# sjtuytc/betapose

Measured on AMD Instinct MI355X. Metric: frames/sec (640x480, 50-kp KPD), higher is better.
Workload: dtype f32 as an exact 3-way bf16 operand split (6 bf16 MFMA products), f32 accumulate and activations

## Files before the change

betapose_amd/_lib.py:

```python
from __future__ import annotations

import ctypes as C
import os
import threading

_HERE = os.path.dirname(os.path.abspath(__file__))
LIB_PATH = os.environ.get("BP_LIB") or os.path.join(_HERE, "libbetapose_hip.so")
_lock = threading.Lock()
_lib = None

c_float_p = C.POINTER(C.c_float)
c_double_p = C.POINTER(C.c_double)
c_int_p = C.POINTER(C.c_int)
vp = C.c_void_p

PROTOTYPES = {
    "bp_last_error": (C.c_char_p, []),
    "bp_version": (C.c_int, []),
    "bp_device_count": (C.c_int, []),
    "bp_device_name": (C.c_int, [C.c_int, C.c_char_p, C.c_int]),
    "bp_yolo_create": (C.c_int, [C.c_char_p, C.c_char_p, C.c_int, C.c_int, C.c_int, C.POINTER(vp)]),
    "bp_yolo_create_from_memory": (C.c_int, [C.c_char_p, vp, C.c_size_t, C.c_int, C.c_int, C.c_int, C.POINTER(vp)]),
    "bp_yolo_clone": (C.c_int, [vp, C.POINTER(vp)]),
    "bp_kpd_clone": (C.c_int, [vp, C.POINTER(vp)]),
# ... 10 lines not shown
    "bp_kpd_destroy": (None, [vp]),
    "bp_kpd_forward": (C.c_int, [vp, vp, C.c_int, vp, vp]),
    "bp_kpd_forward_argmax": (C.c_int, [vp, vp, C.c_int, vp, vp, vp]),
    "bp_kpd_tap_count": (C.c_int, [vp]),
    "bp_kpd_tap_info": (C.c_int, [vp, C.c_int, C.c_char_p, C.c_int, c_int_p, c_int_p, c_int_p]),
    "bp_kpd_tap_copy": (C.c_int, [vp, C.c_int, C.c_int, vp, vp]),
    "bp_yolo_set_policy": (C.c_int, [vp, C.c_int, C.c_int, C.c_int, C.c_int]),
    "bp_kpd_set_policy": (C.c_int, [vp, C.c_int, C.c_int, C.c_int, C.c_int]),
    "bp_yolo_set_precision": (C.c_int, [vp, C.c_int]),
    "bp_kpd_set_precision": (C.c_int, [vp, C.c_int]),
    "bp_calibrate_ticks": (C.c_int, [C.c_longlong, c_float_p, vp]),
    "bp_yolo_set_prefetch": (C.c_int, [vp, C.c_int]),
    "bp_kpd_set_prefetch": (C.c_int, [vp, C.c_int]),
    "bp_yolo_set_fusion": (C.c_int, [vp, C.c_int]),
    "bp_kpd_set_fusion": (C.c_int, [vp, C.c_int]),
    "bp_yolo_fused_launches": (C.c_int, [vp, C.c_int, C.POINTER(C.c_int)]),
    "bp_kpd_fused_launches": (C.c_int, [vp, C.c_int, C.POINTER(C.c_int)]),
    "bp_yolo_xcd_errors": (C.c_int, [vp, C.POINTER(C.c_int), vp]),
    "bp_kpd_xcd_errors": (C.c_int, [vp, C.POINTER(C.c_int), vp]),
    "bp_yolo_set_stamps": (C.c_int, [vp, vp, C.c_int]),
    "bp_kpd_set_stamps": (C.c_int, [vp, vp, C.c_int]),
    "bp_yolo_op_name": (C.c_int, [vp, C.c_int, C.c_char_p, C.c_int]),
    "bp_kpd_op_name": (C.c_int, [vp, C.c_int, C.c_char_p, C.c_int]),
    "bp_yolo_op_stats": (C.c_int, [vp, c_double_p, c_double_p, C.c_int]),
    "bp_kpd_op_stats": (C.c_int, [vp, c_double_p, c_double_p, C.c_int]),
    "bp_yolo_device_bytes": (C.c_size_t, [vp]),
    "bp_kpd_device_bytes": (C.c_size_t, [vp]),
    "bp_crop": (C.c_int, [vp, C.c_int, C.c_int, C.c_int, vp, C.c_int, vp, vp, vp, vp, C.c_int, C.c_int, vp]),
    "bp_resize_bicubic": (C.c_int, [vp, C.c_int, C.c_int, C.c_int, C.c_int, C.c_int, C.c_int, vp, vp, vp]),
    "bp_conv2d": (C.c_int, [vp, C.c_int, C.c_int, C.c_int, C.c_int, vp, vp, C.c_int, C.c_int, C.c_int, C.c_int,
# ... 118 lines not shown
```

betapose_amd/csrc/aux_kernels.hip:

```cpp
#include "bp_common.h"

namespace bp {

__device__ __forceinline__ void store_plane(unsigned short* planes, long long idx, long long plane_elems, int np, float v) {
    if (np == 1) {
        const _Float16 h = (_Float16)v;
        planes[idx] = __builtin_bit_cast(unsigned short, h);
    } else if (np == 3) {
        const __bf16 h1 = (__bf16)v;
        const float r1 = v - (float)h1;
        const __bf16 h2 = (__bf16)r1;
        const __bf16 h3 = (__bf16)(r1 - (float)h2);
        planes[idx] = __builtin_bit_cast(unsigned short, h1);
        planes[idx + plane_elems] = __builtin_bit_cast(unsigned short, h2);
        planes[idx + 2 * plane_elems] = __builtin_bit_cast(unsigned short, h3);
    }
}

static inline int grid_for(long long n, int block = 256, int cap = 4096) {
    BP_CHECK(n < (1ll << 31), "tensor too large for 32-bit indexing");
    long long g = (n + block - 1) / block;
    return (int)(g < 1 ? 1 : (g > cap ? cap : g));
}

// ... 243 lines not shown
        const float stride = (float)(reso / g);
        const float* t = H.t + ((long long)n * g * g + cell) * (3 * attrs) + a * attrs;
        float* o = pred + e * attrs;
        o[0] = (sigmoidf_(t[0]) + (float)gx) * stride;
        o[1] = (sigmoidf_(t[1]) + (float)gy) * stride;
        o[2] = (expf(t[2]) * (H.aw[a] / stride)) * stride;
        o[3] = (expf(t[3]) * (H.ah[a] / stride)) * stride;
        for (int k = 4; k < attrs; ++k) o[k] = sigmoidf_(t[k]);
    }
}
void launch_yolo_decode(const YoloHead* heads, int nheads, int N, int reso, int attrs, int rows, float* pred,
                        hipStream_t s) {
    BP_CHECK(nheads <= 4, "at most 4 yolo heads");
    YoloHeads hs;
    hs.n = nheads;
    for (int i = 0; i < nheads; ++i) hs.h[i] = heads[i];
    hipLaunchKernelGGL(yolo_decode_kernel, dim3(grid_for((long long)N * rows)), dim3(256), 0, s, hs, N, reso, attrs, rows, pred);
}

__global__ __launch_bounds__(1024) void yolo_select_kernel(const float* __restrict__ pred, int rows, int attrs,
                                                            float conf, int num_classes, float* __restrict__ sel, int sel_ld) {
    __shared__ float sv[16];
    __shared__ int si[16];
    const int n = blockIdx.x;
    const float* P = pred + (long long)n * rows * attrs;
    const int ncls = min(num_classes, attrs - 5);
    float best = -1.f;
    int bi = 0x7fffffff;
    for (int r = threadIdx.x; r < rows; r += blockDim.x) {
        const float* q = P + (long long)r * attrs;
        const float obj = q[4];
// ... 32 lines not shown
            o[7] = 0.f;
        }
    }
}
void launch_yolo_select(const float* pred, int N, int rows, int attrs, float conf, int num_classes, float* sel,
                        hipStream_t s, int sel_ld) {
    hipLaunchKernelGGL(yolo_select_kernel, dim3(N), dim3(1024), 0, s, pred, rows, attrs, conf, num_classes, sel, sel_ld);
}

__global__ __launch_bounds__(1024) void yolo_decode_select_kernel(YoloHeads hs, int reso, int attrs, int rows, float conf, int num_classes,
                                                                   float* __restrict__ sel, int sel_ld) {
    __shared__ float sv[16];
    __shared__ int si[16];
    const int n = blockIdx.x;
    const int ncls = min(num_classes, attrs - 5);
    auto locate = [&](int row, int* a) -> const float* {
        int hi = 0;
        for (int k = 1; k < hs.n; ++k)
            if (row >= hs.h[k].row_off) hi = k;
        const YoloHead& H = hs.h[hi];
        const int g = H.g, r = row - H.row_off;
        *a = r / (g * g);
        const int cell = r - *a * g * g;
        return H.t + ((long long)n * g * g + cell) * (3 * attrs) + *a * attrs;
    };
    float best = -1.f;
    int bi = 0x7fffffff;
    for (int r = threadIdx.x; r < rows; r += blockDim.x) {
        int a;
        const float* t = locate(r, &a);
        const float obj = sigmoidf_(t[4]);
        if (!(obj > conf)) continue;
        int cls = 0;
        float cm = sigmoidf_(t[5]);
        for (int k = 1; k < ncls; ++k) {
            const float v = sigmoidf_(t[5 + k]);
            if (v > cm) { cm = v; cls = k; }
        }
        if (cls != 0) continue;
        if (obj > best || (obj == best && r < bi)) { best = obj; bi = r; }
    }
    for (int off = 32; off > 0; off >>= 1) {
        const float ov = __shfl_down(best, off, 64);
        const int oi = __shfl_down(bi, off, 64);
        if (ov > best || (ov == best && oi < bi)) { best = ov; bi = oi; }
    }
    const int w = threadIdx.x >> 6;
    if ((threadIdx.x & 63) == 0) { sv[w] = best; si[w] = bi; }
    __syncthreads();
    if (threadIdx.x == 0) {
        for (int k = 1; k < (int)(blockDim.x >> 6); ++k)
            if (sv[k] > best || (sv[k] == best && si[k] < bi)) { best = sv[k]; bi = si[k]; }
        float* o = sel + (long long)n * sel_ld;
        if (best < 0.f) {
            o[0] = __int_as_float(-1);
            for (int k = 1; k < 8; ++k) o[k] = 0.f;
        } else {
            int a, hi = 0;
            const float* t = locate(bi, &a);
            for (int k = 1; k < hs.n; ++k)
                if (bi >= hs.h[k].row_off) hi = k;
            const YoloHead& H = hs.h[hi];
            const int g = H.g, r = bi - H.row_off, cell = r - a * g * g;
            const int gy = cell / g, gx = cell - gy * g;
            const float stride = (float)(reso / g);
            const float q0 = (sigmoidf_(t[0]) + (float)gx) * stride;
            const float q1 = (sigmoidf_(t[1]) + (float)gy) * stride;
            const float q2 = (expf(t[2]) * (H.aw[a] / stride)) * stride;
            const float q3 = (expf(t[3]) * (H.ah[a] / stride)) * stride;
            o[0] = __int_as_float(bi);
            o[1] = q0 - q2 / 2;
            o[2] = q1 - q3 / 2;
            o[3] = q0 + q2 / 2;
            o[4] = q1 + q3 / 2;
            o[5] = sigmoidf_(t[4]);
            o[6] = sigmoidf_(t[5]);
            o[7] = 0.f;
        }
    }
}
void launch_yolo_decode_select(const YoloHead* heads, int nheads, int N, int reso, int attrs, int rows, float conf, int num_classes,
                               float* sel, hipStream_t s, int sel_ld) {
    BP_CHECK(nheads <= 4, "at most 4 yolo heads");
    YoloHeads hs;
    hs.n = nheads;
    for (int i = 0; i < nheads; ++i) hs.h[i] = heads[i];
    hipLaunchKernelGGL(yolo_decode_select_kernel, dim3(N), dim3(1024), 0, s, hs, reso, attrs, rows, conf, num_classes, sel, sel_ld);
}

__global__ __launch_bounds__(256) void heatmap_argmax_kernel(const float* __restrict__ hm, int H, int W,
                                                              float* __restrict__ out, int C, int out_ld) {
    __shared__ float sv[4];
    __shared__ int si[4];
    const int HW = H * W;
    const float* P = hm + (long long)blockIdx.x * HW;
    float best = -INFINITY;
    int bi = 0x7fffffff;
    for (int i = threadIdx.x; i < HW; i += 256) {
        const float v = P[i];
        if (v > best) { best = v; bi = i; }
    }
// ... 270 lines not shown
```

betapose_amd/csrc/bp_common.h:

```cpp
#pragma once
#include <hip/hip_runtime.h>
#include <cstdint>
#include <cstdio>
#include <mutex>
#include <set>
#include <stdexcept>
#include <string>
#include <utility>

namespace bp {

struct Error : std::runtime_error {
    using std::runtime_error::runtime_error;
};

#define BP_HIP(expr)                                                                      \
    do {                                                                                  \
        hipError_t _e = (expr);                                                           \
        if (_e != hipSuccess)                                                             \
            throw ::bp::Error(std::string(#expr) + ": " + hipGetErrorString(_e) + " @" +  \
                              __FILE__ + ":" + std::to_string(__LINE__));                 \
    } while (0)

#define BP_CHECK(cond, msg)                                                               \
// ... 79 lines not shown
    const unsigned short* wbd;
    const unsigned short* wpl;
    float* pool_out;
    int hy_full, hy_splits, hy_cps;
    int xcd_home;
    int* xcc_of;
    int* err_word;
    int* tickets_local;
    int mtiles, n_tiles;
    int work_blocks;
    const void* pf_ptr;
    int pf_first;
    int pf_ntn, pf_splits, pf_cps, pf_nchunks;
    int pf_tile_stride, pf_chunk_bytes;
    int pf_cap;
};

enum Precision : int { PREC_F32 = 0, PREC_F16 = 1, PREC_BF16X3 = 2, PREC_F16_RES = 3 };

enum ConvTile : int { TILE_64x64 = 0, TILE_128x64 = 1, TILE_W64_1x1 = 2, TILE_W64_1x2 = 3, TILE_W64_2x1 = 5, TILE_W64_2x2 = 6,
                      TILE_KG1 = 7, TILE_KG2 = 8, TILE_KG4 = 9,
                      TILE_RD4 = 10, TILE_RD8 = 11,
                      TILE_64x64_BD = 12,
                      TILE_PL64 = 13,
                      TILE_PL128 = 14,
                      TILE_PL128x64 = 15,
                      TILE_PL256x128 = 16,
                      TILE_STEM3 = 20,
                      TILE_PL64BD = 19,
                      TILE_PL64K2 = 18,
                      TILE_PL128S = 17,
// ... 79 lines not shown
                long long pixels, int C, hipStream_t s);
void launch_upsample2(const float* in, int in_ld, float* out, int out_ld, int N, int H, int W, int C, hipStream_t s);
void launch_copy_channels(const float* in, int in_ld, float* out, int out_ld, long long pixels, int C, hipStream_t s);
void launch_pixel_shuffle2(const float* in, float* out, int N, int H, int W, int C, hipStream_t s,
                           unsigned short* planes = nullptr, long long plane_elems = 0, int np = 0);
int avgpool_parts(int HW);
void launch_avgpool(const float* in, int in_ld, float* out, int N, int HW, int C, hipStream_t s);
void launch_fc(const float* in, const float* w, const float* bias, float* out, int N, int Cin, int Cout,
               int act, int in_parts, float in_scale, hipStream_t s);

struct YoloHead {
    const float* t;
    int g;
    float aw[3], ah[3];
    int row_off;
};
void launch_yolo_decode(const YoloHead* heads, int nheads, int N, int reso, int attrs, int rows,
                        float* pred, hipStream_t s);
void launch_yolo_select(const float* pred, int N, int rows, int attrs, float conf, int num_classes,
                        float* sel, hipStream_t s, int sel_ld = 8);
void launch_yolo_decode_select(const YoloHead* heads, int nheads, int N, int reso, int attrs, int rows, float conf, int num_classes,
                               float* sel, hipStream_t s, int sel_ld = 8);
void launch_heatmap_argmax(const float* hm, int N, int C, int H, int W, float* out, hipStream_t s, int out_ld = 0);

void launch_f32_to_f16(const float* in, unsigned short* out, long long n, hipStream_t s);
void launch_f32_to_bf16x3(const float* in, unsigned short* out_planes, long long n, hipStream_t s);
void launch_f32_to_f16_staged(const float* in, unsigned short* out, int CoutPad, int Kpad, hipStream_t s);
void launch_f32_to_bf16x3_staged(const float* in, unsigned short* out, int CoutPad, int Kpad, hipStream_t s, int Cin_pl = 0);
void launch_probe_placement(int* d_out, int blocks, hipStream_t s);
void launch_spin_ticks(long long ticks, hipStream_t s);
// ... 17 lines not shown
```

betapose_amd/csrc/c_api.cpp:

```cpp
#include "../../include/betapose_hip.h"

#include <algorithm>
#include <cmath>
#include <cstdlib>
#include <cstring>
#include <fstream>
#include <memory>
#include <sstream>
#include <vector>

#include "engine.h"
#include "frame_io.h"

namespace bp {
int solve_pnp(const double* P, const double* U, int n, const double* K, double* R, double* t);
int solve_pnp_refined(const double* P, const double* U, int n, const double* K, double* R, double* t);
int solve_pnp_ransac(const double* P, const double* U, int n, const double* K, double reproj_err, int max_trials,
                     double confidence, double* R, double* t, unsigned char* inlier_mask);
void pnp_ransac_samples(int n, int max_trials, int* idx);
void pnp_ransac_trials_needed(int n, double confidence, int* need);
int pose_nms(const float* bboxes, const float* bbox_scores, const float* preds, const float* scores, int n, int K,
             int* out_pick, float* out_pose, float* out_score, float* out_prop);
int pose_error_blocks(int n);
void launch_pose_errors(const double* model, int n, const double* gt, const double* est, int P, const double* K,
// ... 229 lines not shown
    if (default_precision() != bp::PREC_F32) y->net->set_precision(default_precision());
    *out = y.release();
    return 0;
    BP_CATCH
}

int bp_yolo_clone(const bp_yolo* y, bp_yolo** out) {
    BP_TRY
    BP_CHECK(y && out, "null argument");
    BP_HIP(hipSetDevice(y->device));
    std::unique_ptr<bp_yolo> c(new bp_yolo);
    c->device = y->device;
    c->net.reset(y->net->clone());
    if (y->net->precision() != bp::PREC_F32) c->net->set_precision(y->net->precision_id());
    c->net->set_fusion(y->net->fusion());
    *out = c.release();
    return 0;
    BP_CATCH
}
void bp_yolo_destroy(bp_yolo* y) { delete y; }
int bp_yolo_rows(const bp_yolo* y) { return y ? y->net->rows() : -1; }
int bp_yolo_attrs(const bp_yolo* y) { return y ? y->net->attrs() : -1; }

int bp_yolo_forward(bp_yolo* y, const float* d_img, int batch, float* d_pred, void* stream) {
    BP_TRY
    BP_CHECK(y && d_img && d_pred, "null argument");
    y->net->forward(d_img, false, batch, d_pred, 0.f, 0, nullptr, (hipStream_t)stream);
    return 0;
    BP_CATCH
}
// ... 154 lines not shown
    bp::launch_spin_ticks(1000, s);
    BP_HIP(hipEventRecord(e0, s));
    bp::launch_spin_ticks(ticks, s);
    BP_HIP(hipEventRecord(e1, s));
    BP_HIP(hipEventSynchronize(e1));
    BP_HIP(hipEventElapsedTime(ms, e0, e1));
    (void)hipEventDestroy(e0);
    (void)hipEventDestroy(e1);
    return 0;
    BP_CATCH
}
int bp_yolo_set_prefetch(bp_yolo* y, int on) { y->net->set_prefetch(on != 0); return 0; }
int bp_kpd_set_prefetch(bp_kpd* k, int on) { k->net->set_prefetch(on != 0); return 0; }
int bp_yolo_set_fusion(bp_yolo* y, int on) { y->net->set_fusion(on != 0); return 0; }
int bp_kpd_set_fusion(bp_kpd* k, int on) { k->net->set_fusion(on != 0); return 0; }
int bp_yolo_fused_launches(bp_yolo* y, int batch, int* launches) {
    BP_TRY
    BP_CHECK(y && launches && batch >= 1 && batch <= y->net->max_batch(), "arguments");
    BP_HIP(hipSetDevice(y->device));
    *launches = y->net->fused_launches(batch);
    return 0;
    BP_CATCH
}
int bp_kpd_fused_launches(bp_kpd* k, int batch, int* launches) {
    BP_TRY
    BP_CHECK(k && launches && batch >= 1 && batch <= k->net->max_batch(), "arguments");
    BP_HIP(hipSetDevice(k->device));
    *launches = k->net->fused_launches(batch);
    return 0;
    BP_CATCH
// ... 770 lines not shown
```

betapose_amd/csrc/conv_halo.hip:

```cpp
#include "conv_dev.h"

namespace bp {

static constexpr int HALO_ROW_B = 208;

template <int NW, int NPASS>
__global__ __launch_bounds__(64 * NW) void conv_halo_kernel(const ConvParams p) {
    constexpr int NT = 64 * NW, BM = 64, BN = 32 * NW, TM = 2, TN = 1, LDT = BN + 4;
    constexpr int RPP = NT / 4;
    extern __shared__ __attribute__((aligned(16))) float smem[];
    char* const lds = reinterpret_cast<char*>(smem);

    const unsigned long long t_entry = p.stamps ? bp_clock() : 0ull;
    const int tid = threadIdx.x;
    const int lane = tid & 63;
    const int wave = __builtin_amdgcn_readfirstlane(tid >> 6);
    const int n_tiles_n = p.CoutPad / BN;
    const int split = (int)blockIdx.x % p.splits;
    const int tile_id = (int)blockIdx.x / p.splits;
    const int tile_n = tile_id % n_tiles_n;
    const int tile_m = tile_id / n_tiles_n;
    const int m0 = tile_m * BM, n0 = tile_n * BN;
    const int cpt = p.Cin >> 5;
    const int gps = p.chunks_per_split / 9;
// ... 354 lines not shown
                for (int q = 0; q < 4; ++q) {
                    const f32x4 v = *reinterpret_cast<const f32x4*>(xch + (i * 4 + q) * 256);
                    acc[i][0][4 * q] += v.x; acc[i][0][4 * q + 1] += v.y; acc[i][0][4 * q + 2] += v.z; acc[i][0][4 * q + 3] += v.w;
                }
        }
        __syncthreads();
    }

    const int w_row0 = 0, w_col0 = 32 * wn;
    const bool has_acc = kg == 0;
#define BP_NT NT
#define BP_SLAST (*s_last_p)
#define BP_EARLY_BIAS bias_early
#define BP_HAS_ACC has_acc
#define BP_EP_PIXSHUF
#define BP_TAIL_STAMP(k_) BHK_STAMP(k_)
#include "conv_tail.inc"
#undef BP_EP_PIXSHUF
#undef BP_HAS_ACC
#undef BP_EARLY_BIAS
#undef BP_TAIL_STAMP
#undef BP_NT
#undef BP_SLAST
    if (p.stamps) { asm volatile("s_waitcnt vmcnt(0)" ::: "memory"); BHK_STAMP(4); }
#undef BHK_STAMP
}

template <int NPASS>
__global__ __launch_bounds__(256) void conv_halo_k2_kernel(const ConvParams p) {
    extern __shared__ __attribute__((aligned(16))) float smem[];
    __shared__ int s_last;
    conv_halo_k2_body<NPASS>(p, (int)blockIdx.x, smem, &s_last);
// ... 39 lines not shown
    const size_t lds = conv_halo_lds_bytes(p, tile);
    allow_big_lds(reinterpret_cast<const void*>(&conv_halo_k2_kernel<NPASS>));
    dim3 grid(q.n_tiles * q.splits);
    if (g_conv_prof)
        hipExtLaunchKernelGGL((conv_halo_k2_kernel<NPASS>), grid, dim3(256), lds, s, g_conv_prof->e0, g_conv_prof->e1, 0, q);
    else
        hipLaunchKernelGGL((conv_halo_k2_kernel<NPASS>), grid, dim3(256), lds, s, q);
}

void launch_conv_halo(const ConvParams& p, int tile, hipStream_t s) {
    BP_CHECK(p.mfma_mode == PREC_BF16X3 && conv_halo_eligible(p, tile),
             "halo tile: bf16x3 mode, 3x3 / stride 1 / pad 1, Cin % 32 == 0, stage-packed filters, W <= 95 (64x128) or 79 (64x64)");
    BP_CHECK((long long)3 * p.CoutPad * p.Kpad * 2 < (long long)OOB, "filter planes too large for 32-bit offsets");
    BP_CHECK(p.chunks_per_split % 9 == 0, "halo tile: K slices are whole channel groups (chunks_per_split % 9 == 0)");
    BP_CHECK(!p.xcd_home && !p.pf_ptr && p.hy_splits == 0, "halo tile: no latency-mode layouts");
    const int np = halo_passes(p, tile);
    if (tile == TILE_HALO64K2) {
        switch (np) {
            case 3: launch_halo_k2_t<3>(p, tile, s); break;
            case 4: launch_halo_k2_t<4>(p, tile, s); break;
            case 5: launch_halo_k2_t<5>(p, tile, s); break;
            case 6: launch_halo_k2_t<6>(p, tile, s); break;
            default: launch_halo_k2_t<7>(p, tile, s); break;
        }
    } else if (tile == TILE_HALO128) {
        switch (np) {
            case 2: launch_halo_t<4, 2>(p, tile, s); break;
            case 3: launch_halo_t<4, 3>(p, tile, s); break;
            default: launch_halo_t<4, 4>(p, tile, s); break;
        }
// ... 13 lines not shown
```

betapose_amd/csrc/conv_tail.inc:

```
#ifdef BP_HAS_ACC
    const bool EP_HAS_ACC = BP_HAS_ACC;
#else
    constexpr bool EP_HAS_ACC = true;
#endif
    constexpr int EP_TPR = BN / 4;
    constexpr int EP_ROWS = BP_NT / EP_TPR;
    constexpr int EP_PASSES = BM / EP_ROWS;
#ifndef BP_EP_PF_MAX
#define BP_EP_PF_MAX 4
#define BP_TAIL_OWN_PF_MAX
#endif
    constexpr int EP_PF = EP_PASSES <= BP_EP_PF_MAX ? 1 : 0;
    const int ep_n4 = (tid % EP_TPR) * 4;
    const int ep_n = n0 + ep_n4;
    const int ep_row0 = tid / EP_TPR;
#ifdef BP_EARLY_BIAS
    const f32x4 ep_bias4 = BP_EARLY_BIAS;
#else
    const f32x4 ep_bias4 = *reinterpret_cast<const f32x4*>(p.bias + min(ep_n, p.CoutPad - 4));
#endif
#ifdef BP_EP_PIXSHUF
    const bool ep_ps = p.store_mode == ST_PIXSHUF && p.res == nullptr && ((p.Cout >> 2) & 3) == 0 && p.pool_out == nullptr;
#else
    constexpr bool ep_ps = false;
// ... 159 lines not shown
#pragma unroll
                        for (int r = 0; r < 16; ++r) {
                            const int row = w_row0 - sl * SLAB_ROWS + i * 32 + (r & 3) + 8 * (r >> 2) + 4 * (lane >> 5);
                            smem[row * LDT + w_col0 + j * 32 + (lane & 31)] = acc[i][j][r];
                        }
            }
            __syncthreads();
            if constexpr (EP_SLABS == 1 && BM == 64) {
                if (p.pool_out != nullptr && tid < BN && n0 + tid < p.Cout) {
                    const int nvalid = min(BM, p.M - m0);
                    float s = 0.f;
                    for (int r = 0; r < nvalid; ++r) s += smem[r * LDT + tid];
                    p.pool_out[(long long)(m0 / BM) * p.Cout + n0 + tid] = s + (float)nvalid * p.bias[n0 + tid];
                }
            }
            if (ep_n < p.Cout) {
                const float* srow = &smem[ep_row0 * LDT + ep_n4];
                const unsigned off_o = (unsigned)(((m0 + sl * SLAB_ROWS + ep_row0) * p.out_ld + ep_n) * 4), step_o = (unsigned)(EP_ROWS * p.out_ld * 4);
                const unsigned off_r = ep_off_r + (unsigned)(sl * SLAB_ROWS * p.res_ld * ep_rb);
                PixShufRows ep_rows;
                if (ep_ps) {
                    const int cq = p.Cout >> 2, ij = ep_n / cq, cc = ep_n - ij * cq;
                    ep_rows.m_first = m0 + sl * SLAB_ROWS + ep_row0; ep_rows.m_step = EP_ROWS; ep_rows.M = p.M;
                    ep_rows.hw = p.OH * p.OW; ep_rows.OW = p.OW; ep_rows.OH = p.OH; ep_rows.out_ld = p.out_ld;
                    ep_rows.sub = (unsigned)((((ij >> 1) * (2 * p.OW) + (ij & 1)) * p.out_ld + cc) * 4);
                    ep_rows.rcp_hw = 1.0f / (float)ep_rows.hw; ep_rows.rcp_ow = 1.0f / (float)p.OW;
                }
                Up2Rows ep_uprows;
                if (ep_up) {
                    ep_uprows.m_first = m0 + sl * SLAB_ROWS + ep_row0; ep_uprows.m_step = EP_ROWS; ep_uprows.M = p.M;
// ... 44 lines not shown
```

betapose_amd/csrc/engine.cpp:

```cpp
#include "engine.h"

#include <algorithm>
#include <cmath>
#include <cstdlib>
#include <cstring>
#include <sstream>

namespace bp {

Arena::~Arena() {
    for (void* p : ptrs_) (void)hipFree(p);
}
void* Arena::alloc_bytes(size_t bytes) {
    void* p = nullptr;
    bytes = (bytes + 255) & ~size_t(255);
    BP_HIP(hipMalloc(&p, bytes));
    ptrs_.push_back(p);
    total_ += bytes;
    return p;
}
float* Arena::alloc(size_t n) { return static_cast<float*>(alloc_bytes(n * sizeof(float))); }

Tensor Net::new_tensor(int H, int W, int C) {
    Tensor t;
// ... 1022 lines not shown
#ifdef BP_EXPERIMENTAL
void Net::emit_conv_ops(int batch, std::vector<MegaOp>& out) {
    BP_CHECK(batch >= 1 && batch <= max_batch_, "batch out of range");
    for (const Op& op : ops_) {
        if (op.type != OP_CONV) continue;
        ConvParams p;
        int tile;
        prepare_conv(op, batch, p, tile);
        MegaOp o;
        mega_make_conv_op(p, tile, &o);
        out.push_back(o);
    }
}
#endif

void Net::run_op(const Op& op, int batch, hipStream_t s) {
    if (op.type == OP_CONV) {
        plan_roles(batch);
        const int idx = (int)(&op - ops_.data());
        const int role = roles_[idx];
        if (role == FR_SKIP) return;
        if (role == FR_HEAD2 || role == FR_HEAD3) {
            const FuseGroup& g = fuse_groups_[role_group_[idx]];
            ConvParams a, b, c;
            int ta, tb, tc;
            prepare_conv(ops_[g.pre], batch, a, ta);
            prepare_conv(ops_[g.c3], batch, b, tb);
            if (role == FR_HEAD3) prepare_conv(ops_[g.post], batch, c, tc);
            if (stamps_ && conv_fused_blocks(a, b, role == FR_HEAD3 ? &c : nullptr) > stamp_slots_) b.stamps = c.stamps = nullptr;
            launch_conv_fused(a, b, role == FR_HEAD3 ? &c : nullptr, s);
            return;
        }
    }
    run_op_unfused(op, batch, s);
// ... 100 lines not shown
        }
    }
    return n;
}

void Net::tap_copy(int i, int batch, float* d_out_nchw, hipStream_t s) {
    BP_CHECK(i >= 0 && i < (int)taps_.size(), "tap index");
    const Tensor& t = taps_[i];
    plan_roles(batch);
    for (int j = 0; j < (int)ops_.size(); ++j)
        if (ops_[j].type == OP_CONV && roles_[j] == FR_SKIP && ops_[j].conv.out == t.p) {
            const FuseGroup& g = fuse_groups_[role_group_[j]];
            run_op_unfused(ops_[g.pre], batch, s);
            if (j == g.c3) run_op_unfused(ops_[g.c3], batch, s);
        }
    if (ActAlloc* a = find_act(t.p); a && a->planes && !a->f32_read && precision_ != PREC_F32)
        launch_planes_to_f32(a->planes + (t.p - a->base), (long long)a->elems, precision_ == PREC_F16 ? 1 : 3, t.p, t.ld,
                             (long long)batch * t.H * t.W, t.C, s);
    launch_nhwc_to_nchw(t.p, t.ld, d_out_nchw, batch, t.C, t.H, t.W, s);
    BP_HIP(hipGetLastError());
}

struct CfgBlock {
    std::string type;
    std::map<std::string, std::string> kv;
    bool has(const std::string& k) const { return kv.count(k) != 0; }
    int geti(const std::string& k, int def) const {
        auto it = kv.find(k);
        return it == kv.end() ? def : std::atoi(it->second.c_str());
    }
// ... 220 lines not shown
            BP_CHECK(t.C == 3 * (5 + classes) && t.ld == t.C, "yolo head channel count");
            BP_CHECK(attrs_ == 0 || attrs_ == 5 + classes, "heads disagree on classes");
            attrs_ = 5 + classes;
            YoloHead h{};
            h.t = t.p; h.g = t.H; h.row_off = row_off;
            for (int a = 0; a < 3; ++a) {
                BP_CHECK(mask[a] >= 0 && 2 * mask[a] + 1 < (int)an.size(), "anchor mask");
                h.aw[a] = (float)an[2 * mask[a]];
                h.ah[a] = (float)an[2 * mask[a] + 1];
            }
            heads_.push_back(h);
            row_off += 3 * t.H * t.W;
        }
    }
    BP_CHECK(!heads_.empty() && heads_.size() <= 4, "cfg must have 1..4 yolo layers");
    rows_ = row_off;
    pred_ = arena_.alloc((size_t)max_batch * rows_ * attrs_);
    finalize();
}

void YoloNet::forward(const float* d_img, bool nhwc_input, int batch, float* d_pred, float conf, int num_classes,
                      float* d_sel, hipStream_t s, int sel_ld) {
    BP_CHECK(batch >= 1 && batch <= max_batch_, "batch out of range");
    if (nhwc_input) {
        if (d_img != in_nhwc_)
            BP_HIP(hipMemcpyAsync(in_nhwc_, d_img, (size_t)batch * reso_ * reso_ * 3 * sizeof(float),
                                  hipMemcpyDeviceToDevice, s));
    } else {
        launch_nchw_to_nhwc(d_img, in_nhwc_, batch, 3, reso_, reso_, s);
    }
    run_ops(batch, s);
    static const bool two_kernels = std::getenv("BP_NO_DECODE_FUSION") != nullptr;
    if (d_sel && !d_pred && !two_kernels) {
        launch_yolo_decode_select(heads_.data(), (int)heads_.size(), batch, reso_, attrs_, rows_, conf, num_classes, d_sel, s, sel_ld);
    } else {
        float* pred = d_pred ? d_pred : pred_;
        launch_yolo_decode(heads_.data(), (int)heads_.size(), batch, reso_, attrs_, rows_, pred, s);
        if (d_sel) launch_yolo_select(pred, batch, rows_, attrs_, conf, num_classes, d_sel, s, sel_ld);
    }
    BP_HIP(hipGetLastError());
}

KpdNet::KpdNet(const float* stream, size_t n_floats, int n_classes, int max_batch, int inH, int inW,
               std::shared_ptr<WeightStore> store)
    : Net(max_batch, store), n_floats_(n_floats), n_classes_(n_classes), inH_(inH), inW_(inW) {
    BP_CHECK(inH % 32 == 0 && inW % 32 == 0, "KPD input must be a multiple of 32");
    BP_CHECK(n_classes >= 1, "n_classes");
    outC_ = std::min(n_classes, 50);
    size_t cur = 0;
// ... 168 lines not shown
```

betapose_amd/csrc/engine.h:

```cpp
#pragma once
#include <map>
#include <memory>
#include <mutex>
#include <string>
#include <vector>

#include "bp_common.h"

namespace bp {

struct Tensor {
    float* p = nullptr;
    int H = 0, W = 0, C = 0;
    int ld = 0;
};

class Arena {
public:
    ~Arena();
    float* alloc(size_t n_floats);
    void* alloc_bytes(size_t bytes);
    size_t total_bytes() const { return total_; }
private:
    std::vector<void*> ptrs_;
// ... 58 lines not shown
    int tap_count() const { return (int)taps_.size(); }
    const char* tap_name(int i) const { return tap_names_[i].c_str(); }
    void tap_shape(int i, int* C, int* H, int* W) const { *C = taps_[i].C; *H = taps_[i].H; *W = taps_[i].W; }
    void tap_copy(int i, int batch, float* d_out_nchw, hipStream_t s);
    void set_splitk_policy(int target_blocks, int min_chunks) { sk_target_ = target_blocks; sk_min_chunks_ = min_chunks; ++plan_version_; }
    void set_max_splits(int m) { sk_max_splits_ = m; ++plan_version_; }
    void set_force_tile(int t) { force_tile_ = t; ++plan_version_; }
    void set_precision(int prec);
    int precision() const { return precision_; }
    int precision_id() const { return (precision_ == PREC_F16 && f16_res_) ? PREC_F16_RES : precision_; }
    unsigned plan_version() const { return plan_version_; }
    void set_stamps(unsigned long long* d_buf, int slots) { stamps_ = d_buf; stamp_slots_ = slots; ++plan_version_; }
    void set_prefetch(bool on) { prefetch_ = on; ++plan_version_; }
    void set_fusion(bool on) { fusion_ = on; ++plan_version_; }
    bool fusion() const { return fusion_; }
    int fused_launches(int batch);
    int take_xcd_errors(hipStream_t s);
    bool pool_in_epilogue(const Op& conv, int batch, int tile) const;
    bool pooled_by_conv(const Op& pool, int batch) const;
    bool prefetch() const { return prefetch_; }
    const char* op_name(int i) const { return ops_[i].name.c_str(); }

protected:
    int add_conv(const std::string& name, const Tensor& in, const Tensor& out_view, const ConvWeights& cw, int Cout,
                 int k, int stride, int pad, int act, int store_mode, const Tensor* res, const float* res_scale,
                 int res_after_act, float bn_eps, int OH, int OW);
    void add_tap(const std::string& name, const Tensor& t) { taps_.push_back(t); tap_names_.push_back(name); }
    Tensor new_tensor(int H, int W, int C);
    void finalize();
    size_t workspace_need() const;
// ... 21 lines not shown
    bool darknet_bn_ = false;
    int precision_ = PREC_F32;
    unsigned long long* stamps_ = nullptr;
    int stamp_slots_ = 0;
    bool prefetch_ = false;
    struct FuseGroup { int pre, c3, post; };
    enum FuseRole : int { FR_NONE = 0, FR_SKIP = 1, FR_HEAD2 = 2, FR_HEAD3 = 3 };
    std::vector<FuseGroup> fuse_groups_;
    std::vector<int> roles_, role_group_;
    int roles_batch_ = -1;
    unsigned roles_version_ = ~0u;
    bool fusion_ = true;
    void find_fuse_groups();
    void plan_roles(int batch);
    void run_op_unfused(const Op& op, int batch, hipStream_t s);
    bool f16_res_ = false;
    unsigned plan_version_ = 0;
};

class YoloNet : public Net {
public:
    YoloNet(const std::string& cfg_text, const float* stream, size_t n_floats, int reso, int max_batch,
            std::shared_ptr<WeightStore> store = nullptr, bool darknet_bn = false);
    YoloNet* clone() const { return new YoloNet(cfg_text_, nullptr, n_floats_, reso_, max_batch_, store_, darknet_bn_); }
    int rows() const { return rows_; }
    int attrs() const { return attrs_; }
    int reso() const { return reso_; }
    void forward(const float* d_img, bool nhwc_input, int batch, float* d_pred, float conf, int num_classes,
                 float* d_sel, hipStream_t s, int sel_ld = 8);
    float* input_nhwc() { return in_nhwc_; }
// ... 39 lines not shown
```

betapose_amd/darknet.py:

```python
from __future__ import annotations

import ctypes as C
import os
from typing import Optional

import numpy as np

from . import _lib
from .cfg import parse_cfg, parse_cfg_text, yolov3_single_cfg_text
from .weights import darknet_stream_size, read_darknet_weights


def _cfg_text(blocks) -> str:
    out = []
    for b in blocks:
        out.append("[%s]" % b["type"])
        for k, v in b.items():
            if k != "type":
                out.append("%s=%s" % (k, v))
        out.append("")
    return "\n".join(out)


class Darknet:
# ... 146 lines not shown
        info = (C.c_int * (4 * n))()
        rc = L.bp_yolo_profile(self._h, batch, iters, ms, info, n, _lib.current_stream())
        if rc < 0:
            _lib.check(rc)
        return np.array(ms, dtype=np.float64), np.array(info, dtype=np.int64).reshape(n, 4)

    def set_prefetch(self, on: bool = True):
        self._ensure()
        _lib.check(_lib.lib().bp_yolo_set_prefetch(self._h, int(bool(on))))
        self._latency_mode = bool(on)

    def set_fusion(self, on: bool = True):
        self._ensure()
        _lib.check(_lib.lib().bp_yolo_set_fusion(self._h, int(bool(on))))

    def fused_launches(self, batch: int = 1) -> int:
        self._ensure()
        n = C.c_int(0)
        _lib.check(_lib.lib().bp_yolo_fused_launches(self._h, int(batch), C.byref(n)))
        return int(n.value)

    def xcd_errors(self) -> int:
        if not getattr(self, "_latency_mode", False) or self._h is None:
            return 0
        n = C.c_int(0)
        _lib.check(_lib.lib().bp_yolo_xcd_errors(self._h, C.byref(n), _lib.current_stream()))
        return int(n.value)

    def set_stamps(self, buf=None, slots: int = 0):
        self._ensure()
# ... 33 lines not shown
```

include/betapose_hip.h:

```cpp
#ifndef BETAPOSE_HIP_H
#define BETAPOSE_HIP_H

#include <stddef.h>
#include <stdint.h>

#ifdef __cplusplus
extern "C" {
#endif

typedef struct bp_yolo bp_yolo;
typedef struct bp_kpd bp_kpd;
typedef struct bp_pipeline bp_pipeline;

#define BP_RESULT_FLOATS 316
#define BP_KP_FLOATS 6
#define BP_SEL_FLOATS 8

#define BP_POSE_DOUBLES 166
#define BP_PNP_MAX_POINTS 64

const char* bp_last_error(void);
int bp_version(void);
int bp_device_count(void);
int bp_device_name(int device, char* out, int cap);
// ... 23 lines not shown
int bp_kpd_tap_info(const bp_kpd* k, int i, char* name, int cap, int* C, int* H, int* W);
int bp_kpd_tap_copy(bp_kpd* k, int i, int batch, float* d_out_nchw, void* stream);

int bp_yolo_set_policy(bp_yolo* y, int sk_target_blocks, int sk_min_chunks, int sk_max_splits, int force_tile);
int bp_kpd_set_policy(bp_kpd* k, int sk_target_blocks, int sk_min_chunks, int sk_max_splits, int force_tile);
int bp_yolo_set_precision(bp_yolo* y, int precision);
int bp_kpd_set_precision(bp_kpd* k, int precision);
int bp_yolo_op_stats(const bp_yolo* y, double* flops, double* bytes, int cap);
int bp_kpd_op_stats(const bp_kpd* k, double* flops, double* bytes, int cap);
int bp_yolo_profile(bp_yolo* y, int batch, int iters, float* ms, int* info, int cap, void* stream);
int bp_calibrate_ticks(long long ticks, float* ms, void* stream);
int bp_yolo_set_prefetch(bp_yolo* y, int on);
int bp_kpd_set_prefetch(bp_kpd* k, int on);
int bp_yolo_set_fusion(bp_yolo* y, int on);
int bp_kpd_set_fusion(bp_kpd* k, int on);
int bp_yolo_fused_launches(bp_yolo* y, int batch, int* launches);
int bp_kpd_fused_launches(bp_kpd* k, int batch, int* launches);
int bp_yolo_xcd_errors(bp_yolo* y, int* count, void* stream);
int bp_kpd_xcd_errors(bp_kpd* k, int* count, void* stream);
int bp_yolo_set_stamps(bp_yolo* y, unsigned long long* d_buf, int slots);
int bp_kpd_set_stamps(bp_kpd* k, unsigned long long* d_buf, int slots);
int bp_yolo_op_name(const bp_yolo* y, int i, char* out, int cap);
int bp_kpd_op_name(const bp_kpd* k, int i, char* out, int cap);
int bp_kpd_profile(bp_kpd* k, int batch, int iters, float* ms, int* info, int cap, void* stream);
size_t bp_yolo_device_bytes(const bp_yolo* y);
size_t bp_kpd_device_bytes(const bp_kpd* k);

int bp_crop(const uint8_t* d_frames, int batch, int H, int W, const float* d_sel, int reso, const float* d_boxes,
            float* d_out_nchw, float* d_out_nhwc, float* d_pts, int oh, int ow, void* stream);
int bp_resize_bicubic(const uint8_t* d_in, int batch, int H, int W, int oh, int ow, int swap_rb, uint8_t* d_out_u8,
// ... 91 lines not shown
```

Before: 993.7.

## Fold YOLO 1x1 head convs into producer 3x3 conv epilogue

Each YOLO head's 1x1 linear conv is fused into the epilogue of the preceding 3x3 conv. The epilogue multiplies the activated tile by packed head weights and writes per-N-tile partial sums. The decode/select kernel then sums those partials plus bias, so the producer's full activation tensor is never stored and the head conv launches are removed. It applies only at batch 1 with bf16x3 precision and the 64x64 halo K2 tile. In exchange the epilogue does extra FMAs and the select kernel makes extra strided reads.

Result: slower. 916.7 (-7.7%).

```diff
diff --git a/betapose_amd/_lib.py b/betapose_amd/_lib.py
--- a/betapose_amd/_lib.py
+++ b/betapose_amd/_lib.py
@@ -48,6 +48,8 @@
     "bp_kpd_set_prefetch": (C.c_int, [vp, C.c_int]),
     "bp_yolo_set_fusion": (C.c_int, [vp, C.c_int]),
     "bp_kpd_set_fusion": (C.c_int, [vp, C.c_int]),
+    "bp_yolo_set_head_fold": (C.c_int, [vp, C.c_int]),
+    "bp_pack_head_filters": (C.c_int, [vp, C.c_int, C.c_int, vp]),
     "bp_yolo_fused_launches": (C.c_int, [vp, C.c_int, C.POINTER(C.c_int)]),
     "bp_kpd_fused_launches": (C.c_int, [vp, C.c_int, C.POINTER(C.c_int)]),
     "bp_yolo_xcd_errors": (C.c_int, [vp, C.POINTER(C.c_int), vp]),
diff --git a/betapose_amd/csrc/aux_kernels.hip b/betapose_amd/csrc/aux_kernels.hip
--- a/betapose_amd/csrc/aux_kernels.hip
+++ b/betapose_amd/csrc/aux_kernels.hip
@@ -281,7 +281,10 @@
     BP_CHECK(nheads <= 4, "at most 4 yolo heads");
     YoloHeads hs;
     hs.n = nheads;
-    for (int i = 0; i < nheads; ++i) hs.h[i] = heads[i];
+    for (int i = 0; i < nheads; ++i) {
+        hs.h[i] = heads[i];
+        BP_CHECK(heads[i].part == nullptr, "yolo_decode reads the head tensors: no folded heads on this path");
+    }
     hipLaunchKernelGGL(yolo_decode_kernel, dim3(grid_for((long long)N * rows)), dim3(256), 0, s, hs, N, reso, attrs, rows, pred);
 }
 
@@ -344,27 +347,40 @@
     __shared__ int si[16];
     const int n = blockIdx.x;
     const int ncls = min(num_classes, attrs - 5);
-    auto locate = [&](int row, int* a) -> const float* {
+    struct Loc { int hi, a, cell; };
+    auto locate = [&](int row) -> Loc {
         int hi = 0;
         for (int k = 1; k < hs.n; ++k)
             if (row >= hs.h[k].row_off) hi = k;
-        const YoloHead& H = hs.h[hi];
-        const int g = H.g, r = row - H.row_off;
-        *a = r / (g * g);
-        const int cell = r - *a * g * g;
-        return H.t + ((long long)n * g * g + cell) * (3 * attrs) + *a * attrs;
+        const int g = hs.h[hi].g, r = row - hs.h[hi].row_off;
+        const int a = r / (g * g);
+        return Loc{hi, a, r - a * g * g};
+    };
+    auto val = [&](const Loc& L, int k) -> float {
+        const YoloHead& H = hs.h[L.hi];
+        const int g = H.g;
+        if (H.part == nullptr) return H.t[((long long)n * g * g + L.cell) * (3 * attrs) + L.a * attrs + k];
+        const int c = L.a * attrs + k, ts = g * g * HEAD_NP;
+        const float* q = H.part + L.cell * HEAD_NP + c;
+        float s = 0.f;
+        int tn = 0;
+        for (; tn + 4 <= H.ntn; tn += 4) {
+            const float v0 = q[tn * ts], v1 = q[(tn + 1) * ts], v2 = q[(tn + 2) * ts], v3 = q[(tn + 3) * ts];
+            s = (((s + v0) + v1) + v2) + v3;
+        }
+        for (; tn < H.ntn; ++tn) s += q[tn * ts];
+        return s + H.bias[c];
     };
     float best = -1.f;
     int bi = 0x7fffffff;
     for (int r = threadIdx.x; r < rows; r += blockDim.x) {
-        int a;
-        const float* t = locate(r, &a);
-        const float obj = sigmoidf_(t[4]);
+        const Loc L = locate(r);
+        const float obj = sigmoidf_(val(L, 4));
         if (!(obj > conf)) continue;
         int cls = 0;
-        float cm = sigmoidf_(t[5]);
+        float cm = sigmoidf_(val(L, 5));
         for (int k = 1; k < ncls; ++k) {
-            const float v = sigmoidf_(t[5 + k]);
+            const float v = sigmoidf_(val(L, 5 + k));
             if (v > cm) { cm = v; cls = k; }
         }
         if (cls != 0) continue;
@@ -386,25 +402,22 @@
             o[0] = __int_as_float(-1);
             for (int k = 1; k < 8; ++k) o[k] = 0.f;
         } else {
-            int a, hi = 0;
-            const float* t = locate(bi, &a);
-            for (int k = 1; k < hs.n; ++k)
-                if (bi >= hs.h[k].row_off) hi = k;
-            const YoloHead& H = hs.h[hi];
-            const int g = H.g, r = bi - H.row_off, cell = r - a * g * g;
+            const Loc L = locate(bi);
+            const YoloHead& H = hs.h[L.hi];
+            const int g = H.g, a = L.a, cell = L.cell;
             const int gy = cell / g, gx = cell - gy * g;
             const float stride = (float)(reso / g);
-            const float q0 = (sigmoidf_(t[0]) + (float)gx) * stride;
-            const float q1 = (sigmoidf_(t[1]) + (float)gy) * stride;
-            const float q2 = (expf(t[2]) * (H.aw[a] / stride)) * stride;
-            const float q3 = (expf(t[3]) * (H.ah[a] / stride)) * stride;
+            const float q0 = (sigmoidf_(val(L, 0)) + (float)gx) * stride;
+            const float q1 = (sigmoidf_(val(L, 1)) + (float)gy) * stride;
+            const float q2 = (expf(val(L, 2)) * (H.aw[a] / stride)) * stride;
+            const float q3 = (expf(val(L, 3)) * (H.ah[a] / stride)) * stride;
             o[0] = __int_as_float(bi);
             o[1] = q0 - q2 / 2;
             o[2] = q1 - q3 / 2;
             o[3] = q0 + q2 / 2;
             o[4] = q1 + q3 / 2;
-            o[5] = sigmoidf_(t[4]);
-            o[6] = sigmoidf_(t[5]);
+            o[5] = sigmoidf_(val(L, 4));
+            o[6] = sigmoidf_(val(L, 5));
             o[7] = 0.f;
         }
     }
@@ -414,7 +427,10 @@
     BP_CHECK(nheads <= 4, "at most 4 yolo heads");
     YoloHeads hs;
     hs.n = nheads;
-    for (int i = 0; i < nheads; ++i) hs.h[i] = heads[i];
+    for (int i = 0; i < nheads; ++i) {
+        hs.h[i] = heads[i];
+        BP_CHECK(heads[i].part == nullptr || (N == 1 && 3 * attrs <= HEAD_NP && heads[i].bias != nullptr && heads[i].ntn >= 1), "folded yolo head: batch 1, at most HEAD_NP channels");
+    }
     hipLaunchKernelGGL(yolo_decode_select_kernel, dim3(N), dim3(1024), 0, s, hs, reso, attrs, rows, conf, num_classes, sel, sel_ld);
 }
 
diff --git a/betapose_amd/csrc/bp_common.h b/betapose_amd/csrc/bp_common.h
--- a/betapose_amd/csrc/bp_common.h
+++ b/betapose_amd/csrc/bp_common.h
@@ -117,7 +117,12 @@
     int pf_ntn, pf_splits, pf_cps, pf_nchunks;
     int pf_tile_stride, pf_chunk_bytes;
     int pf_cap;
-};
+    const float* head_w = nullptr;
+    float* head_part = nullptr;
+};
+
+constexpr int HEAD_NP = 20;
+void pack_head_filters(const float* w, int Cout, int Cin, float* out);
 
 enum Precision : int { PREC_F32 = 0, PREC_F16 = 1, PREC_BF16X3 = 2, PREC_F16_RES = 3 };
 
@@ -227,6 +232,9 @@
     int g;
     float aw[3], ah[3];
     int row_off;
+    const float* part = nullptr;
+    const float* bias = nullptr;
+    int ntn = 0;
 };
 void launch_yolo_decode(const YoloHead* heads, int nheads, int N, int reso, int attrs, int rows,
                         float* pred, hipStream_t s);
diff --git a/betapose_amd/csrc/c_api.cpp b/betapose_amd/csrc/c_api.cpp
--- a/betapose_amd/csrc/c_api.cpp
+++ b/betapose_amd/csrc/c_api.cpp
@@ -267,6 +267,7 @@
     c->net.reset(y->net->clone());
     if (y->net->precision() != bp::PREC_F32) c->net->set_precision(y->net->precision_id());
     c->net->set_fusion(y->net->fusion());
+    c->net->set_head_fold(y->net->head_fold());
     *out = c.release();
     return 0;
     BP_CATCH
@@ -451,6 +452,14 @@
 int bp_kpd_set_prefetch(bp_kpd* k, int on) { k->net->set_prefetch(on != 0); return 0; }
 int bp_yolo_set_fusion(bp_yolo* y, int on) { y->net->set_fusion(on != 0); return 0; }
 int bp_kpd_set_fusion(bp_kpd* k, int on) { k->net->set_fusion(on != 0); return 0; }
+int bp_yolo_set_head_fold(bp_yolo* y, int on) { y->net->set_head_fold(on != 0); return 0; }
+int bp_pack_head_filters(const float* w, int Cout, int Cin, float* out) {
+    BP_TRY
+    BP_CHECK(w && out && Cout >= 1 && Cout <= bp::HEAD_NP && Cin >= 1, "arguments");
+    bp::pack_head_filters(w, Cout, Cin, out);
+    return 0;
+    BP_CATCH
+}
 int bp_yolo_fused_launches(bp_yolo* y, int batch, int* launches) {
     BP_TRY
     BP_CHECK(y && launches && batch >= 1 && batch <= y->net->max_batch(), "arguments");
diff --git a/betapose_amd/csrc/conv_halo.hip b/betapose_amd/csrc/conv_halo.hip
--- a/betapose_amd/csrc/conv_halo.hip
+++ b/betapose_amd/csrc/conv_halo.hip
@@ -392,8 +392,10 @@
 #define BP_EARLY_BIAS bias_early
 #define BP_HAS_ACC has_acc
 #define BP_EP_PIXSHUF
+#define BP_EP_HEAD
 #define BP_TAIL_STAMP(k_) BHK_STAMP(k_)
 #include "conv_tail.inc"
+#undef BP_EP_HEAD
 #undef BP_EP_PIXSHUF
 #undef BP_HAS_ACC
 #undef BP_EARLY_BIAS
@@ -463,6 +465,10 @@
     BP_CHECK((long long)3 * p.CoutPad * p.Kpad * 2 < (long long)OOB, "filter planes too large for 32-bit offsets");
     BP_CHECK(p.chunks_per_split % 9 == 0, "halo tile: K slices are whole channel groups (chunks_per_split % 9 == 0)");
     BP_CHECK(!p.xcd_home && !p.pf_ptr && p.hy_splits == 0, "halo tile: no latency-mode layouts");
+    BP_CHECK(p.head_w == nullptr || (tile == TILE_HALO64K2 && p.head_part != nullptr && p.Cout % 64 == 0 && p.store_mode == ST_NHWC && p.res == nullptr &&
+                                     p.res_scale == nullptr && p.pool_out == nullptr && p.out16 == nullptr && (p.out_ld & 3) == 0 &&
+                                     conv_halo_lds_bytes(p, tile) >= (size_t)4 * 64 * HEAD_NP * 4),
+             "halo tile: a folded head needs the 64x64 K2 tile and a plain NHWC epilogue");
     const int np = halo_passes(p, tile);
     if (tile == TILE_HALO64K2) {
         switch (np) {
diff --git a/betapose_amd/csrc/conv_tail.inc b/betapose_amd/csrc/conv_tail.inc
--- a/betapose_amd/csrc/conv_tail.inc
+++ b/betapose_amd/csrc/conv_tail.inc
@@ -197,6 +197,37 @@
                     p.pool_out[(long long)(m0 / BM) * p.Cout + n0 + tid] = s + (float)nvalid * p.bias[n0 + tid];
                 }
             }
+#ifdef BP_EP_HEAD
+            if (p.head_w != nullptr) {
+                static_assert(BN == 64 && BP_NT == 256 && BM == 64, "head fold: 64x64 tile, four waves");
+                const int hrow = tid & 63, hk0 = wave * 16;
+                const float* hwp = p.head_w + (long long)(n0 + hk0) * HEAD_NP;
+                const float* hbp = p.bias + n0 + hk0;
+                float hacc[HEAD_NP];
+#pragma unroll
+                for (int c = 0; c < HEAD_NP; ++c) hacc[c] = 0.f;
+#pragma unroll
+                for (int kk = 0; kk < 16; kk += 4) {
+                    const f32x4 a4 = *reinterpret_cast<const f32x4*>(&smem[hrow * LDT + hk0 + kk]);
+#pragma unroll
+                    for (int u = 0; u < 4; ++u) {
+                        const float a = apply_act(a4[u] + hbp[kk + u], p.act);
+#pragma unroll
+                        for (int c = 0; c < HEAD_NP; ++c) hacc[c] = fmaf(a, hwp[(kk + u) * HEAD_NP + c], hacc[c]);
+                    }
+                }
+                __syncthreads();
+                float* hq = smem + (wave * 64 + hrow) * HEAD_NP;
+#pragma unroll
+                for (int c = 0; c < HEAD_NP; c += 4) *reinterpret_cast<f32x4*>(hq + c) = f32x4{hacc[c], hacc[c + 1], hacc[c + 2], hacc[c + 3]};
+                __syncthreads();
+                const int hn = min(BM, p.M - m0) * HEAD_NP;
+                float* hdst = p.head_part + ((long long)tile_n * p.M + m0) * HEAD_NP;
+                for (int e = tid; e < hn; e += BP_NT)
+                    hdst[e] = ((smem[e] + smem[64 * HEAD_NP + e]) + smem[2 * 64 * HEAD_NP + e]) + smem[3 * 64 * HEAD_NP + e];
+                return;
+            }
+#endif
             if (ep_n < p.Cout) {
                 const float* srow = &smem[ep_row0 * LDT + ep_n4];
                 const unsigned off_o = (unsigned)(((m0 + sl * SLAB_ROWS + ep_row0) * p.out_ld + ep_n) * 4), step_o = (unsigned)(EP_ROWS * p.out_ld * 4);
diff --git a/betapose_amd/csrc/engine.cpp b/betapose_amd/csrc/engine.cpp
--- a/betapose_amd/csrc/engine.cpp
+++ b/betapose_amd/csrc/engine.cpp
@@ -1060,10 +1060,41 @@
 }
 #endif
 
+void pack_head_filters(const float* w, int Cout, int Cin, float* out) {
+    for (int ci = 0; ci < Cin; ++ci)
+        for (int c = 0; c < HEAD_NP; ++c) out[(size_t)ci * HEAD_NP + c] = c < Cout ? w[(size_t)c * Cin + ci] : 0.f;
+}
+
+bool Net::head_folds_apply(int batch) {
+    static const bool env_off = std::getenv("BP_NO_HEAD_FOLD") != nullptr;
+    if (head_folds_.empty() || !head_fold_ || env_off || batch != 1 || precision_ != PREC_BF16X3 || force_tile_ >= 0 || stamps_ || prefetch_) return false;
+    plan_roles(batch);
+    for (const HeadFold& f : head_folds_) {
+        if (roles_[f.prod] != FR_NONE || roles_[f.head] != FR_NONE) return false;
+        ConvParams p;
+        int tile;
+        prepare_conv(ops_[f.prod], batch, p, tile);
+        if (tile != TILE_HALO64K2 || p.pool_out || p.out16 || p.hy_splits || ops_[f.head].conv.in16) return false;
+    }
+    return true;
+}
+
 void Net::run_op(const Op& op, int batch, hipStream_t s) {
     if (op.type == OP_CONV) {
         plan_roles(batch);
         const int idx = (int)(&op - ops_.data());
+        if (head_fold_now_)
+            for (const HeadFold& f : head_folds_) {
+                if (idx == f.head) return;
+                if (idx == f.prod) {
+                    ConvParams p;
+                    int tile;
+                    prepare_conv(op, batch, p, tile);
+                    p.head_w = f.w; p.head_part = f.part;
+                    launch_conv(p, tile, s);
+                    return;
+                }
+            }
         const int role = roles_[idx];
         if (role == FR_SKIP) return;
         if (role == FR_HEAD2 || role == FR_HEAD3) {
@@ -1194,6 +1225,12 @@
             run_op_unfused(ops_[g.pre], batch, s);
             if (j == g.c3) run_op_unfused(ops_[g.c3], batch, s);
         }
+    if (head_fold_last_)
+        for (const HeadFold& f : head_folds_)
+            if (ops_[f.prod].conv.out == t.p || ops_[f.head].conv.out == t.p) {
+                run_op_unfused(ops_[f.prod], batch, s);
+                if (ops_[f.head].conv.out == t.p) run_op_unfused(ops_[f.head], batch, s);
+            }
     if (ActAlloc* a = find_act(t.p); a && a->planes && !a->f32_read && precision_ != PREC_F32)
         launch_planes_to_f32(a->planes + (t.p - a->base), (long long)a->elems, precision_ == PREC_F16 ? 1 : 3, t.p, t.ld,
                              (long long)batch * t.H * t.W, t.C, s);
@@ -1444,6 +1481,36 @@
         }
     }
     BP_CHECK(!heads_.empty() && heads_.size() <= 4, "cfg must have 1..4 yolo layers");
+    for (int h = 0; h < (int)heads_.size(); ++h)
+        for (int j = 1; j < (int)ops_.size(); ++j) {
+            if (ops_[j].type != OP_CONV || ops_[j].conv.out != heads_[h].t || ops_[j - 1].type != OP_CONV) continue;
+            const ConvParams& hc = ops_[j].conv;
+            const ConvParams& pc = ops_[j - 1].conv;
+            if (!(hc.ksize == 1 && hc.stride == 1 && hc.act == ACT_LINEAR && hc.res == nullptr && hc.store_mode == ST_NHWC && hc.Cout <= HEAD_NP &&
+                  hc.in == pc.out && hc.in_ld == pc.out_ld && hc.Cin == pc.Cout)) continue;
+            if (!(pc.ksize == 3 && pc.stride == 1 && pc.pad == 1 && pc.res == nullptr && pc.res_scale == nullptr && pc.store_mode == ST_NHWC &&
+                  pc.Cout % 64 == 0 && pc.out_ld == pc.Cout)) continue;
+            int readers = 0;
+            for (const Op& o : ops_) {
+                if (o.type == OP_CONV) readers += (o.conv.in == pc.out) + (o.conv.res == pc.out);
+                else readers += (o.a == pc.out) + (o.b == pc.out);
+            }
+            if (readers != 1) continue;
+            HeadFold f{j - 1, j, h, nullptr, nullptr, pc.Cout / 64};
+            if (reuse_) {
+                f.w = upload_weights(nullptr, 0);
+            } else {
+                std::vector<float> hw((size_t)hc.Cin * hc.Cout), packed((size_t)hc.Cin * HEAD_NP);
+                std::vector<float> full((size_t)hc.CoutPad * hc.Kpad);
+                BP_HIP(hipMemcpy(full.data(), hc.w, full.size() * sizeof(float), hipMemcpyDeviceToHost));
+                for (int co = 0; co < hc.Cout; ++co)
+                    for (int ci = 0; ci < hc.Cin; ++ci) hw[(size_t)co * hc.Cin + ci] = full[(size_t)co * hc.Kpad + ci];
+                pack_head_filters(hw.data(), hc.Cout, hc.Cin, packed.data());
+                f.w = upload_weights(packed.data(), packed.size());
+            }
+            f.part = arena_.alloc((size_t)f.ntn * hc.OH * hc.OW * HEAD_NP);
+            head_folds_.push_back(f);
+        }
     rows_ = row_off;
     pred_ = arena_.alloc((size_t)max_batch * rows_ * attrs_);
     finalize();
@@ -1459,10 +1526,17 @@
     } else {
         launch_nchw_to_nhwc(d_img, in_nhwc_, batch, 3, reso_, reso_, s);
     }
-    run_ops(batch, s);
     static const bool two_kernels = std::getenv("BP_NO_DECODE_FUSION") != nullptr;
+    const bool fold = d_sel && !d_pred && !two_kernels && 3 * attrs_ <= HEAD_NP && head_folds_.size() == heads_.size() && head_folds_apply(batch);
+    head_fold_now_ = fold;
+    try { run_ops(batch, s); } catch (...) { head_fold_now_ = false; throw; }
+    head_fold_now_ = false;
+    head_fold_last_ = fold;
     if (d_sel && !d_pred && !two_kernels) {
-        launch_yolo_decode_select(heads_.data(), (int)heads_.size(), batch, reso_, attrs_, rows_, conf, num_classes, d_sel, s, sel_ld);
+        std::vector<YoloHead> hv = heads_;
+        if (fold)
+            for (const HeadFold& f : head_folds_) { hv[f.yolo].part = f.part; hv[f.yolo].bias = ops_[f.head].conv.bias; hv[f.yolo].ntn = f.ntn; }
+        launch_yolo_decode_select(hv.data(), (int)heads_.size(), batch, reso_, attrs_, rows_, conf, num_classes, d_sel, s, sel_ld);
     } else {
         float* pred = d_pred ? d_pred : pred_;
         launch_yolo_decode(heads_.data(), (int)heads_.size(), batch, reso_, attrs_, rows_, pred, s);
diff --git a/betapose_amd/csrc/engine.h b/betapose_amd/csrc/engine.h
--- a/betapose_amd/csrc/engine.h
+++ b/betapose_amd/csrc/engine.h
@@ -96,6 +96,8 @@
     void set_prefetch(bool on) { prefetch_ = on; ++plan_version_; }
     void set_fusion(bool on) { fusion_ = on; ++plan_version_; }
     bool fusion() const { return fusion_; }
+    void set_head_fold(bool on) { head_fold_ = on; ++plan_version_; }
+    bool head_fold() const { return head_fold_; }
     int fused_launches(int batch);
     int take_xcd_errors(hipStream_t s);
     bool pool_in_epilogue(const Op& conv, int batch, int tile) const;
@@ -147,6 +149,12 @@
     void find_fuse_groups();
     void plan_roles(int batch);
     void run_op_unfused(const Op& op, int batch, hipStream_t s);
+    struct HeadFold { int prod, head, yolo; float* w; float* part; int ntn; };
+    std::vector<HeadFold> head_folds_;
+    bool head_fold_ = true;
+    bool head_fold_now_ = false;
+    bool head_fold_last_ = false;
+    bool head_folds_apply(int batch);
     bool f16_res_ = false;
     unsigned plan_version_ = 0;
 };
diff --git a/betapose_amd/darknet.py b/betapose_amd/darknet.py
--- a/betapose_amd/darknet.py
+++ b/betapose_amd/darknet.py
@@ -184,6 +184,10 @@
         self._ensure()
         _lib.check(_lib.lib().bp_yolo_set_fusion(self._h, int(bool(on))))
 
+    def set_head_fold(self, on: bool = True):
+        self._ensure()
+        _lib.check(_lib.lib().bp_yolo_set_head_fold(self._h, int(bool(on))))
+
     def fused_launches(self, batch: int = 1) -> int:
         self._ensure()
         n = C.c_int(0)
diff --git a/include/betapose_hip.h b/include/betapose_hip.h
--- a/include/betapose_hip.h
+++ b/include/betapose_hip.h
@@ -61,6 +61,8 @@
 int bp_kpd_set_prefetch(bp_kpd* k, int on);
 int bp_yolo_set_fusion(bp_yolo* y, int on);
 int bp_kpd_set_fusion(bp_kpd* k, int on);
+int bp_yolo_set_head_fold(bp_yolo* y, int on);
+int bp_pack_head_filters(const float* w, int Cout, int Cin, float* out);
 int bp_yolo_fused_launches(bp_yolo* y, int batch, int* launches);
 int bp_kpd_fused_launches(bp_kpd* k, int batch, int* launches);
 int bp_yolo_xcd_errors(bp_yolo* y, int* count, void* stream);
```
